# juliantos/solid-dsp

Measured on AMD Instinct MI355X. Metric: Msamples/sec 256-tap complex FIR @1/2/4/8 GPU; % HBM roofline, higher is better.
Workload: dtype c32 (f32 taps x complex-f32 samples, f32 accumulate); 1 GPU; cfg2: 256-tap crcf FIR, firdes_kaiser(256, 0.1, 80), scale 0.2, 2^30 samples per channel, device resident; parallelism=channels sharded, independent per GPU x 1

## Files before the change

### solid_dsp_amd/csrc/kern_fir_ols_os.hip

```cpp
#include "sdsp_device.hpp"
#include "sdsp_kernels.hpp"
#include "sdsp_pk.hpp"

namespace sdsp {

using namespace pk;

namespace {

constexpr int kRow = 272;

typedef unsigned int u2v __attribute__((ext_vector_type(2)));
typedef unsigned int u4v __attribute__((ext_vector_type(4)));
constexpr int kBufWord3 = 0x00020000;
constexpr int kNT = 2;

__device__ __forceinline__ void wave_sync() {
    __builtin_amdgcn_fence(__ATOMIC_RELEASE, "wavefront");
    __builtin_amdgcn_wave_barrier();
    __builtin_amdgcn_fence(__ATOMIC_ACQUIRE, "wavefront");
}

__device__ __forceinline__ f2 tw_pair(const f2 (&c)[3], const f2 (&d)[3], int k) {
    const int a = k >> 2, b = k & 3;
    if (a == 0) return b == 0 ? f2{1.0f, 0.0f} : c[b - 1];
    if (b == 0) return d[a - 1];
    return pmul(d[a - 1], c[b - 1]);
}

__device__ __forceinline__ void pair_exchange(f2 a, f2 b, f2& lo, f2& hi) {
    float l0, l1, h0, h1;
    asm("s_nop 1\n\t"
        "s_mov_b32 vcc_lo, 0x55555555\n\t"
        "s_mov_b32 vcc_hi, 0x55555555\n\t"
        "v_cndmask_b32_dpp %0, %6, %4, vcc quad_perm:[1,0,3,2] row_mask:0xf bank_mask:0xf\n\t"
        "v_cndmask_b32_dpp %1, %7, %5, vcc quad_perm:[1,0,3,2] row_mask:0xf bank_mask:0xf\n\t"
        "s_not_b64 vcc, vcc\n\t"
        "v_cndmask_b32_dpp %2, %4, %6, vcc quad_perm:[1,0,3,2] row_mask:0xf bank_mask:0xf\n\t"
        "v_cndmask_b32_dpp %3, %5, %7, vcc quad_perm:[1,0,3,2] row_mask:0xf bank_mask:0xf"
        : "=&v"(l0), "=&v"(l1), "=&v"(h0), "=&v"(h1)
        : "v"(a.x), "v"(a.y), "v"(b.x), "v"(b.y)
        : "vcc");
    lo = f2{l0, l1};
    hi = f2{h0, h1};
}

}

template <bool HALO1, bool WIDE, bool EDGE>
__device__ __forceinline__ void ols_os_segment(const f2* __restrict__ xw, const f2* __restrict__ hist,
                                               f2* __restrict__ new_hist, const float4* __restrict__ Hs,
                                               const float4* __restrict__ tb, f2* __restrict__ yw, long long base,
                                               long long n, int Lm1, int h2, f2* img, int t) {
    const int hi4 = t >> 4, lo4 = t & 15;
    if constexpr (HALO1) h2 = 1;
    int nrec = 32768;
    if constexpr (EDGE) {
        const long long rem = n - base;
        if (rem < 4096) nrec = (int)(8 * rem);
    }
    const auto rx = __builtin_amdgcn_make_buffer_rsrc((void*)xw, (short)0, nrec, kBufWord3);
    const auto ry = __builtin_amdgcn_make_buffer_rsrc((void*)yw, (short)0, nrec, kBufWord3);
    const auto rt = __builtin_amdgcn_make_buffer_rsrc((void*)tb, (short)0, kOlsOsTabF4 * 16, kBufWord3);
    const auto rh = __builtin_amdgcn_make_buffer_rsrc((void*)Hs, (short)0, 2048 * 16, kBufWord3);
    const float4 cd = __builtin_bit_cast(float4, __builtin_amdgcn_raw_buffer_load_b128(rt, 16 * t, 16 * kOlsOsTabCD, 0));
    const float4 ef = __builtin_bit_cast(float4, __builtin_amdgcn_raw_buffer_load_b128(rt, 16 * lo4, 16 * kOlsOsTabEF, 0));
    f2 v[16];
    if constexpr (EDGE) {
        const auto rp = __builtin_amdgcn_make_buffer_rsrc((void*)hist, (short)0, 8 * Lm1, kBufWord3);
#pragma unroll
        for (int r = 0; r < 16; ++r) {
            const long long pos = base + 256 * r;
            if (pos >= 0) {
                v[r] = __builtin_bit_cast(f2, __builtin_amdgcn_raw_buffer_load_b64(rx, 8 * t, 2048 * r, 0));
            } else {
                const long long e = Lm1 + pos + t;
                v[r] = __builtin_bit_cast(f2, __builtin_amdgcn_raw_buffer_load_b64(rp, e >= 0 ? (int)(8 * e) : 0x7ffffff0, 0, 0));
            }
        }
        if (new_hist != nullptr) {
            const long long h0 = n - Lm1;
#pragma unroll
            for (int r = 0; r < 16; ++r) {
                const long long i = base + 256 * r + t - h0;
                if (i >= 0 && i < Lm1) new_hist[i] = v[r];
            }
        }
    } else if constexpr (WIDE) {
        f4v q[8];
#pragma unroll
        for (int k = 0; k < 8; ++k)
            q[k] = __builtin_bit_cast(f4v, __builtin_amdgcn_raw_buffer_load_b128(rx, 16 * (t >> 1) + 16384 * (t & 1),
                                                                                2048 * k, kNT));
#pragma unroll
        for (int k = 0; k < 8; ++k) pair_exchange(f2{q[k].x, q[k].y}, f2{q[k].z, q[k].w}, v[k], v[8 + k]);
    } else {
#pragma unroll
        for (int r = 0; r < 16; ++r) {
            if (HALO1 && (r == 0 || r == 15))
                v[r] = __builtin_bit_cast(f2, __builtin_amdgcn_raw_buffer_load_b64(rx, 8 * t, 2048 * r, 0));
            else
                v[r] = __builtin_bit_cast(f2, __builtin_amdgcn_raw_buffer_load_b64(rx, 8 * t, 2048 * r, kNT));
        }
    }
    f2 Cb[3], Da[3], Eb[3], Fa[3];
    {
        const f2 c1 = f2{cd.x, cd.y}, d1 = f2{cd.z, cd.w}, e1 = f2{ef.x, ef.y}, f1 = f2{ef.z, ef.w};
        const f2 c2 = pmul(c1, c1), d2 = pmul(d1, d1), e2 = pmul(e1, e1), f2_ = pmul(f1, f1);
        Cb[0] = c1, Cb[1] = c2, Cb[2] = pmul(c2, c1);
        Da[0] = d1, Da[1] = d2, Da[2] = pmul(d2, d1);
        Eb[0] = e1, Eb[1] = e2, Eb[2] = pmul(e2, e1);
        Fa[0] = f1, Fa[1] = f2_, Fa[2] = pmul(f2_, f1);
    }
    f2* col = img + t + (t >> 4);

    pdft16f<false>(v);
#pragma unroll
    for (int k = 0; k < 16; ++k) col[k * kRow] = k == 0 ? v[0] : pmul(v[kout(k)], tw_pair(Cb, Da, k));
    __syncthreads();

    f2* r2 = img + hi4 * kRow + lo4;
#pragma unroll
    for (int j = 0; j < 16; ++j) v[j] = r2[17 * j];
    float4 hq[8];
#pragma unroll
    for (int p = 0; p < 8; ++p) hq[p] = __builtin_bit_cast(float4, __builtin_amdgcn_raw_buffer_load_b128(rh, 16 * t, 4096 * p, 0));
    f2 w2[16];
#pragma unroll
    for (int k = 1; k < 16; ++k) w2[k] = tw_pair(Eb, Fa, k);
    pdft16f<false>(v);
#pragma unroll
    for (int k = 0; k < 16; ++k) r2[17 * k] = k == 0 ? v[0] : pmul(v[kout(k)], w2[k]);
    wave_sync();

    {
        f2* r3 = img + hi4 * kRow + 17 * lo4;
#pragma unroll
        for (int j = 0; j < 16; ++j) v[j] = r3[j];
        pdft16f<false>(v);
        f2 u[16];
#pragma unroll
        for (int p = 0; p < 8; ++p) {
            u[2 * p] = pmul(v[kout(2 * p)], f2{hq[p].x, hq[p].y});
            u[2 * p + 1] = pmul(v[kout(2 * p + 1)], f2{hq[p].z, hq[p].w});
        }
        pdft16f<true>(u);
#pragma unroll
        for (int j = 0; j < 16; ++j) r3[j] = j == 0 ? u[kout(0)] : pmulc(u[kout(j)], w2[j]);
    }
    wave_sync();

#pragma unroll
    for (int j = 0; j < 16; ++j) v[j] = r2[17 * j];
    pdft16f<true>(v);
#pragma unroll
    for (int k = 0; k < 16; ++k) r2[17 * k] = v[kout(k)];
    __syncthreads();

#pragma unroll
    for (int i = 0; i < 3; ++i) asm volatile("" : "+v"(Cb[i]), "+v"(Da[i]));
#pragma unroll
    for (int k = 0; k < 16; ++k) v[k] = k == 0 ? col[0] : pmulc(col[k * kRow], tw_pair(Cb, Da, k));
    pdft16f<true>(v);
    if constexpr (WIDE && !EDGE) {
#pragma unroll
        for (int k = 0; k < 8; ++k) {
            f2 a, b;
            pair_exchange(v[kout(k)], v[kout(8 + k)], a, b);
            if (k + 8 * (t & 1) >= h2)
                __builtin_amdgcn_raw_buffer_store_b128(__builtin_bit_cast(u4v, f4v{a.x, a.y, b.x, b.y}), ry,
                                                       16 * (t >> 1) + 16384 * (t & 1), 2048 * k, kNT);
        }
    } else {
#pragma unroll
        for (int r = 0; r < 16; ++r)
            if (r >= h2) __builtin_amdgcn_raw_buffer_store_b64(__builtin_bit_cast(u2v, v[kout(r)]), ry, 8 * t, 2048 * r, kNT);
    }
}

template <bool HALO1, bool WIDE, bool EDGE>
__global__ void __launch_bounds__(256, 4)
fir_ols_os_kernel(const f2* __restrict__ x, f2* __restrict__ y, const float4* __restrict__ Hs,
                  const float4* __restrict__ tb, long long stride, unsigned lo, unsigned hi, unsigned q, int h2) {
    static_assert(!EDGE, "the boundary segments take the long argument list");
    __shared__ __attribute__((aligned(16))) f2 img[16 * kRow];
    const unsigned seg = lo + (blockIdx.x & 7u) * q + (blockIdx.x >> 3);
    if (seg >= hi) return;
    if constexpr (HALO1) h2 = 1;
    const unsigned H = 256u * (unsigned)h2;
    const long long off = (long long)((unsigned long long)seg * (4096u - H)) - (long long)H +
                          (long long)blockIdx.y * stride;
    ols_os_segment<HALO1, WIDE, false>(x + off, nullptr, nullptr, Hs, tb, y + off, 0, 0, 0, h2, img, threadIdx.x);
}

template <bool HALO1, bool WIDE, bool EDGE>
__global__ void __launch_bounds__(256, 4)
fir_ols_os_kernel(const f2* __restrict__ x, const f2* __restrict__ hist, f2* __restrict__ new_hist,
                  const float4* __restrict__ Hs, const float4* __restrict__ tb, f2* __restrict__ y, long long n,
                  long long lo, long long hi, long long nseg, int h2, int Lm1) {
    static_assert(EDGE && !HALO1 && !WIDE, "the interior segments take the short argument list");
    __shared__ __attribute__((aligned(16))) f2 img[16 * kRow];
    const long long seg = (long long)blockIdx.x < lo ? (long long)blockIdx.x : hi + ((long long)blockIdx.x - lo);
    const int V = 4096 - 256 * h2;
    const long long ch = blockIdx.y;
    const long long base = seg * V - 256 * h2;
    ols_os_segment<false, false, true>(x + ch * n + base, hist + ch * Lm1,
                                       (new_hist != nullptr && seg == nseg - 1) ? new_hist + ch * Lm1 : nullptr, Hs, tb,
                                       y + ch * n + base, base, n, Lm1, h2, img, threadIdx.x);
}

template <bool HALO1, bool WIDE>
hipError_t launch_fir_ols_os_t(const OlsPlan& p, const void* x, const void* hist, void* new_hist, void* y, size_t n,
                               int Lm1, size_t channels, hipStream_t s) {
    if (n == 0) return hipSuccess;
    const int h2 = p.halo_rows;
    if (h2 < 1 || h2 > 15 || Lm1 > 256 * h2 || (HALO1 && h2 != 1)) return hipErrorInvalidValue;
    const long long V = 4096 - 256 * h2;
    const long long nseg = ((long long)n + V - 1) / V;
    if (nseg >= (1LL << 31)) return hipErrorInvalidValue;
    long long lo, hi;
    ols_interior_range((long long)n, h2, &lo, &hi);
    if (hi > nseg - 1) hi = nseg - 1;
    if (hi < lo) hi = lo;
    const long long nedge = lo + (nseg - hi);
    const long long q = (hi - lo + 7) / 8;
    hipLaunchKernelGGL((fir_ols_os_kernel<false, false, true>), dim3((unsigned)nedge, (unsigned)channels), dim3(256),
                       0, s, (const f2*)x, (const f2*)hist, (f2*)new_hist, (const float4*)p.d_pkt,
                       (const float4*)p.d_ostab, (f2*)y, (long long)n, lo, hi, nseg, h2, Lm1);
    hipError_t e = hipGetLastError();
    if (e != hipSuccess || hi <= lo) return e;
    hipLaunchKernelGGL((fir_ols_os_kernel<HALO1, WIDE, false>), dim3((unsigned)(8 * q), (unsigned)channels), dim3(256),
                       0, s, (const f2*)x, (f2*)y, (const float4*)p.d_pkt, (const float4*)p.d_ostab, (long long)n,
                       (unsigned)lo, (unsigned)hi, (unsigned)q, h2);
    return hipGetLastError();
}

hipError_t launch_fir_ols_os(const OlsPlan& p, const void* x, const void* hist, void* new_hist, void* y, size_t n,
                             int Lm1, size_t channels, hipStream_t s, bool wide) {
    if (wide) return launch_fir_ols_os_t<false, true>(p, x, hist, new_hist, y, n, Lm1, channels, s);
    if (p.halo_rows == 1) return launch_fir_ols_os_t<true, false>(p, x, hist, new_hist, y, n, Lm1, channels, s);
    return launch_fir_ols_os_t<false, false>(p, x, hist, new_hist, y, n, Lm1, channels, s);
}

}
```

### solid_dsp_amd/csrc/runtime.cpp

```cpp
#include <hip/hip_runtime.h>

#include <algorithm>
#include <atomic>
#include <cctype>
#include <cmath>
#include <cstdlib>
#include <cstring>
#include <mutex>
#include <string>
#include <vector>

#include "sdsp.h"
#include "sdsp_host.hpp"
#include "sdsp_kernels.hpp"

namespace sdsp {

static thread_local std::string g_last_error;
void set_error(const std::string& msg) { g_last_error = msg; }

static std::atomic<int> g_default_algo{-1};
static int parse_algo_env(const char* e) {
    if (!e) return SDSP_ALGO_EXACT;
    std::string v(e);
    for (auto& ch : v) ch = (char)std::tolower((unsigned char)ch);
    if (v == "auto" || v == "0") return SDSP_ALGO_AUTO;
    if (v == "fma" || v == "2") return SDSP_ALGO_FMA;
    return SDSP_ALGO_EXACT;
}
int default_algo() {
    int v = g_default_algo.load();
    if (v >= 0) return v;
    int expect = -1;
    g_default_algo.compare_exchange_strong(expect, parse_algo_env(std::getenv("SDSP_DEFAULT_ALGO")));
    return g_default_algo.load();
}
int device_status(hipError_t e, const char* what) {
    if (e == hipSuccess) return SDSP_OK;
    set_error(std::string(what) + ": " + hipGetErrorString(e));
    return e == hipErrorOutOfMemory ? SDSP_E_OUT_OF_MEMORY : SDSP_E_DEVICE;
}
#define SDSP_TRY(expr, what)                              \
    do {                                                  \
        hipError_t _e = (expr);                           \
        if (_e != hipSuccess) return device_status(_e, what); \
    } while (0)

struct DeviceInfo {
    bool ok = false;
    int cus = 256;
};

static int check_device(int device, DeviceInfo* info) {
    int count = 0;
    if (hipGetDeviceCount(&count) != hipSuccess || count <= 0) {
        set_error("no HIP device visible (libsdsp has no CPU execution path)");
        return SDSP_E_NO_DEVICE;
    }
    if (device < 0 || device >= count) {
        set_error("device index out of range");
        return SDSP_E_NO_DEVICE;
    }
    hipDeviceProp_t prop;
    if (hipGetDeviceProperties(&prop, device) != hipSuccess) {
        set_error("hipGetDeviceProperties failed");
        return SDSP_E_NO_DEVICE;
    }
    if (std::strncmp(prop.gcnArchName, "gfx950", 6) != 0) {
        set_error(std::string("libsdsp is built for gfx950; device is ") + prop.gcnArchName);
        return SDSP_E_NO_DEVICE;
    }
    info->ok = true;
    info->cus = prop.multiProcessorCount;
    return SDSP_OK;
}

struct DeviceGuard {
    int prev = -1;
    explicit DeviceGuard(int d) {
        (void)hipGetDevice(&prev);
        if (prev != d) (void)hipSetDevice(d);
    }
    ~DeviceGuard() {
        int cur = -1;
        (void)hipGetDevice(&cur);
        if (prev >= 0 && cur != prev) (void)hipSetDevice(prev);
    }
};

static hipStream_t pick(void* user, hipStream_t own) { return user ? (hipStream_t)user : own; }

}

using namespace sdsp;

struct sdsp_fir {
    int dtype = 0, device = 0, cus = 256;
    mutable unsigned long long device_ops = 0;
    size_t L = 0, M = 1, channels = 1;
    std::vector<unsigned char> taps;
    std::vector<unsigned char> scale;
    DevBuf d_taps_rev;
    DevBuf d_hist[2];
    int cur = 0;
    size_t ci = 0;
    int algo = SDSP_ALGO_EXACT;
    hipStream_t stream = nullptr;
    mutable StreamFence fence;
    DevBuf stage_in, stage_out;
    HostMapped step_out;
    unsigned step_seq = 0;
    std::vector<unsigned char> hbuf;
    size_t hpos = 0;
    bool host_valid = false;
    bool dev_stale = false;
    int host_step = 1;
    size_t host_macs = 1u << 16;
    bool ols_ok = false;
    int ols_kernel = kOlsOneShot;
    int decim_seg = 0;
    OlsPlan ols{};
    DevBuf d_H, d_tw1, d_tw2, d_pkt, d_ostab, d_hhalf;
};

namespace {

int fir_alloc_state(sdsp_fir* h) {
    SDSP_TRY(h->fence.wait(), "wait for queued work");
    const size_t hb = h->channels * (h->L - 1) * sample_bytes(h->dtype);
    for (int i = 0; i < 2; ++i) {
        SDSP_TRY(h->d_hist[i].ensure(hb), "alloc history");
        if (hb) SDSP_TRY(hipMemsetAsync(h->d_hist[i].p, 0, hb, h->stream), "zero history");
    }
    h->cur = 0;
    h->ci = 0;
    SDSP_TRY(hipStreamSynchronize(h->stream), "sync");
    const size_t lm1 = h->L - 1, sb = sample_bytes(h->dtype);
    h->hbuf.assign(2 * lm1 * sb, 0);
    h->hpos = 0;
    h->host_valid = h->channels == 1;
    h->dev_stale = false;
    return SDSP_OK;
}

bool ols_real(const sdsp_fir* h) { return h->dtype == SDSP_RR32; }

bool ols_applicable(const sdsp_fir* h) {
    return (h->dtype == SDSP_RR32 || h->dtype == SDSP_RC32 || h->dtype == SDSP_CC32) && h->M == 1 && h->L >= 2 &&
           h->L - 1 <= 256 * 15;
}

int ols_build(sdsp_fir* h) {
    SDSP_TRY(h->fence.wait(), "wait for queued work");
    const int N = kOlsN;
    const size_t L = h->L;
    const int h2 = (int)((L - 1 + 255) / 256);
    std::vector<cd> g(N, cd{0.0, 0.0});
    const cd s = coef_at(h->scale.data(), h->dtype, 0);
    for (size_t i = 0; i < L; ++i) {
        cd c = coef_at(h->taps.data(), h->dtype, L - 1 - i);
        g[i] = coef_is_complex(h->dtype) ? cmul(c, s) : cd{c.re * s.re, c.re * s.im};
    }
    std::vector<cd> G(N);
    const double w = -2.0 * M_PI / N;
    for (int k = 0; k < N; ++k) {
        double re = 0.0, im = 0.0;
        for (size_t i = 0; i < L; ++i) {
            const long long ph = ((long long)i * k) % N;
            const double c = std::cos(w * (double)ph), sn = std::sin(w * (double)ph);
            re += g[i].re * c - g[i].im * sn;
            im += g[i].re * sn + g[i].im * c;
        }
        G[k] = {re / N, im / N};
    }
    std::vector<float> Hs(2 * 4096), tw1(2 * 4096), tw2(2 * 256);
    for (int t = 0; t < 256; ++t) {
        const int k0 = t >> 4, k1 = t & 15;
        for (int k2 = 0; k2 < 16; ++k2) {
            const cd v = G[k0 + 16 * k1 + 256 * k2];
            Hs[2 * (t * 16 + k2)] = (float)v.re;
            Hs[2 * (t * 16 + k2) + 1] = (float)v.im;
        }
        for (int k = 0; k < 16; ++k) {
            const long long ph = ((long long)t * k) % 4096;
            tw1[2 * (t * 16 + k)] = (float)std::cos(-2.0 * M_PI * ph / 4096.0);
            tw1[2 * (t * 16 + k) + 1] = (float)std::sin(-2.0 * M_PI * ph / 4096.0);
        }
    }
    for (int a = 0; a < 16; ++a)
        for (int b = 0; b < 16; ++b) {
            const int ph = (a * b) % 256;
            tw2[2 * (a * 16 + b)] = (float)std::cos(-2.0 * M_PI * ph / 256.0);
            tw2[2 * (a * 16 + b) + 1] = (float)std::sin(-2.0 * M_PI * ph / 256.0);
        }
    const bool real = ols_real(h);
    if (!real) {
        SDSP_TRY(h->d_H.ensure(Hs.size() * 4), "alloc H");
        SDSP_TRY(h->d_tw1.ensure(tw1.size() * 4), "alloc tw1");
        SDSP_TRY(h->d_tw2.ensure(tw2.size() * 4), "alloc tw2");
        SDSP_TRY(hipMemcpyAsync(h->d_H.p, Hs.data(), Hs.size() * 4, hipMemcpyHostToDevice, h->stream), "copy H");
        SDSP_TRY(hipMemcpyAsync(h->d_tw1.p, tw1.data(), tw1.size() * 4, hipMemcpyHostToDevice, h->stream),
                 "copy tw1");
        SDSP_TRY(hipMemcpyAsync(h->d_tw2.p, tw2.data(), tw2.size() * 4, hipMemcpyHostToDevice, h->stream),
                 "copy tw2");
    }
    std::vector<float> pkt(4 * 4224);
    for (int q = 0; q < 8; ++q) {
        for (int i = 0; i < 256; ++i)
            for (int e = 0; e < 4; ++e) {
                pkt[4 * (q * 256 + i) + e] = Hs[2 * (i * 16 + 2 * q) + e];
                pkt[4 * (2048 + q * 256 + i) + e] = tw1[2 * (i * 16 + 2 * q) + e];
            }
        for (int i = 0; i < 16; ++i)
            for (int e = 0; e < 4; ++e) pkt[4 * (4096 + q * 16 + i) + e] = tw2[2 * (i * 16 + 2 * q) + e];
    }
    SDSP_TRY(h->d_pkt.ensure(pkt.size() * 4), "alloc packed tables");
    SDSP_TRY(hipMemcpyAsync(h->d_pkt.p, pkt.data(), pkt.size() * 4, hipMemcpyHostToDevice, h->stream),
             "copy packed tables");
    std::vector<float> os(4 * kOlsOsTabF4);
    auto put = [&](size_t f4, int half, long long m, int nn) {
        const double ang = -2.0 * M_PI * (double)(m % nn) / nn;
        os[4 * f4 + 2 * half] = (float)std::cos(ang);
        os[4 * f4 + 2 * half + 1] = (float)std::sin(ang);
    };
    for (int c = 0; c < 256; ++c) {
        put(c, 0, c, 4096);
        put(c, 1, 2LL * c, 4096);
        put(256 + c, 0, 3LL * c, 4096);
        put(256 + c, 1, 4LL * c, 4096);
        put(512 + c, 0, 8LL * c, 4096);
        put(512 + c, 1, 12LL * c, 4096);
    }
    for (int c = 0; c < 256; ++c) {
        put(kOlsOsTabCD + c, 0, c, 4096);
        put(kOlsOsTabCD + c, 1, 4LL * c, 4096);
    }
    for (int l = 0; l < 16; ++l) {
        put(kOlsOsTabEF + l, 0, l, 256);
        put(kOlsOsTabEF + l, 1, 4LL * l, 256);
    }
    for (int l = 0; l < 16; ++l) {
        put(768 + l, 0, l, 256);
        put(768 + l, 1, 2LL * l, 256);
        put(784 + l, 0, 3LL * l, 256);
        put(784 + l, 1, 4LL * l, 256);
        put(800 + l, 0, 8LL * l, 256);
        put(800 + l, 1, 12LL * l, 256);
    }
    SDSP_TRY(h->d_ostab.ensure(os.size() * 4), "alloc one-shot tables");
    SDSP_TRY(hipMemcpyAsync(h->d_ostab.p, os.data(), os.size() * 4, hipMemcpyHostToDevice, h->stream),
             "copy one-shot tables");
    const bool real_taps = !coef_is_complex(h->dtype) && !real;
    if (real_taps) {
        std::vector<float> hh(4 * 4 * kOlsHalfRow);
        auto set = [&](int q, int i, int half, cd v) {
            hh[4 * (q * kOlsHalfRow + i) + 2 * half] = (float)v.re;
            hh[4 * (q * kOlsHalfRow + i) + 2 * half + 1] = (float)v.im;
        };
        for (int q = 0; q < 4; ++q) {
            for (int i = 0; i < 256; ++i) {
                const int k0 = i >> 4, k1 = i & 15;
                set(q, i, 0, G[k0 + 16 * k1 + 256 * (2 * q)]);
                set(q, i, 1, G[k0 + 16 * k1 + 256 * (2 * q + 1)]);
            }
            const int pp = 7 - q;
            const cd a = G[256 * (2 * pp + 1)], b = G[256 * (2 * pp)];
            set(q, 256, 0, cd{a.re, -a.im});
            set(q, 256, 1, cd{b.re, -b.im});
        }
        SDSP_TRY(h->d_hhalf.ensure(hh.size() * 4), "alloc half spectrum");
        SDSP_TRY(hipMemcpyAsync(h->d_hhalf.p, hh.data(), hh.size() * 4, hipMemcpyHostToDevice, h->stream),
                 "copy half spectrum");
    }
    SDSP_TRY(hipStreamSynchronize(h->stream), "sync");
    h->ols = OlsPlan{};
    h->ols.d_hhalf = real_taps ? h->d_hhalf.p : nullptr;
    h->ols.d_H = real ? nullptr : h->d_H.p;
    h->ols.d_tw1 = real ? nullptr : h->d_tw1.p;
    h->ols.d_tw2 = real ? nullptr : h->d_tw2.p;
    h->ols.sample_bytes = real ? 4 : 8;
    h->ols.halo_rows = h2;
    h->ols.kernel = h->ols_kernel;
    h->ols.d_pkt = h->d_pkt.p;
    h->ols.d_ostab = h->d_ostab.p;
    h->ols_ok = true;
    return SDSP_OK;
}

int fir_resolve_algo(const sdsp_fir* h, size_t n) {
    if (h->algo == SDSP_ALGO_FFT) return ols_applicable(h) ? SDSP_ALGO_FFT : SDSP_ALGO_EXACT;
    if (h->algo != SDSP_ALGO_AUTO) return h->algo;
    if (ols_applicable(h) && !ols_real(h) && n >= (size_t)(1 << 16)) return SDSP_ALGO_FFT;
    return SDSP_ALGO_EXACT;
}
static int decim_resolve_algo(const sdsp_fir* h, size_t n) {
    if (h->algo != SDSP_ALGO_AUTO) return h->algo;
    return h->dtype <= SDSP_CC32 && n >= (size_t)(1 << 16) ? SDSP_ALGO_FMA : SDSP_ALGO_EXACT;
}

int fir_create_common(sdsp_fir** out, int dtype, const void* taps, size_t len, const void* scale, size_t M,
                      int device) {
    *out = nullptr;
    if (dtype < 0 || dtype > 5) {
        set_error("bad dtype");
        return SDSP_E_INVALID_ARGUMENT;
    }
    if (len == 0) {
        set_error("FIR Filter Error CoefficientsLengthZero");
        return SDSP_E_COEFFICIENTS_LENGTH_ZERO;
    }
    if (M < 1) {
        set_error("FIR Filter Error DecimationLessThanOne");
        return SDSP_E_DECIMATION_LESS_THAN_ONE;
    }
    if (len > (1u << 30)) {
        set_error("tap count too large");
        return SDSP_E_INVALID_ARGUMENT;
    }
    DeviceInfo info;
    int st = check_device(device, &info);
    if (st) return st;
    DeviceGuard g(device);
    sdsp_fir* h = new sdsp_fir();
    h->dtype = dtype;
    h->device = device;
    h->algo = default_algo();
    h->cus = info.cus;
    h->L = len;
    h->M = M;
    const size_t cb = coef_bytes(dtype);
    h->taps.assign((const unsigned char*)taps, (const unsigned char*)taps + len * cb);
    h->scale.assign((const unsigned char*)scale, (const unsigned char*)scale + cb);
    std::vector<unsigned char> rev(len * cb);
    for (size_t i = 0; i < len; ++i) std::memcpy(&rev[i * cb], &h->taps[(len - 1 - i) * cb], cb);
    hipError_t e = hipStreamCreateWithFlags(&h->stream, hipStreamNonBlocking);
    if (e == hipSuccess) e = h->d_taps_rev.ensure(rev.size());
    if (e == hipSuccess) e = hipMemcpy(h->d_taps_rev.p, rev.data(), rev.size(), hipMemcpyHostToDevice);
    if (e != hipSuccess) {
        st = device_status(e, "fir create");
        sdsp_fir_destroy(h);
        return st;
    }
    st = fir_alloc_state(h);
    if (st) {
        sdsp_fir_destroy(h);
        return st;
    }
    *out = h;
    return SDSP_OK;
}

}

namespace {
template <typename T> struct hcx {
    T re, im;
};
template <typename T> inline T hmul(T a, T b) { return a * b; }
template <typename T> inline hcx<T> hmul(T a, hcx<T> b) { return {a * b.re, a * b.im}; }
template <typename T> inline hcx<T> hmul(hcx<T> a, T b) { return {a.re * b, a.im * b}; }
template <typename T> inline hcx<T> hmul(hcx<T> a, hcx<T> b) {
    return {a.re * b.re - a.im * b.im, a.re * b.im + a.im * b.re};
}
template <typename T> inline T hadd(T a, T b) { return a + b; }
template <typename T> inline hcx<T> hadd(hcx<T> a, hcx<T> b) { return {a.re + b.re, a.im + b.im}; }
inline float hfma(float acc, float c, float x) { return std::fma(c, x, acc); }
inline double hfma(double acc, double c, double x) { return std::fma(c, x, acc); }
template <typename T> inline hcx<T> hfma(hcx<T> acc, T c, hcx<T> x) { return {hfma(acc.re, c, x.re), hfma(acc.im, c, x.im)}; }
template <typename T> inline hcx<T> hfma(hcx<T> acc, hcx<T> c, hcx<T> x) {
    return {hfma(hfma(acc.re, c.re, x.re), -c.im, x.im), hfma(hfma(acc.im, c.re, x.im), c.im, x.re)};
}
template <typename T> inline T hzero() { return T{}; }

template <typename C, typename I>
void host_step_t(sdsp_fir* h, const unsigned char* sample, unsigned char* out, bool emit, bool fused) {
    const size_t L = h->L, lm1 = L - 1;
    I x;
    std::memcpy(&x, sample, sizeof(I));
    I* b = reinterpret_cast<I*>(h->hbuf.data());
    if (emit) {
        const I* w = b + h->hpos;
        const C* taps = reinterpret_cast<const C*>(h->taps.data());
        I acc = hzero<I>();
        if (fused) {
            acc = hfma(acc, taps[L - 1], x);
            for (size_t i = 1; i < L; ++i) acc = hfma(acc, taps[L - 1 - i], w[lm1 - i]);
        } else {
            acc = hadd(acc, hmul(taps[L - 1], x));
            for (size_t i = 1; i < L; ++i) acc = hadd(acc, hmul(taps[L - 1 - i], w[lm1 - i]));
        }
        C sc;
        std::memcpy(&sc, h->scale.data(), sizeof(C));
        const I y = hmul(acc, sc);
        std::memcpy(out, &y, sizeof(I));
    }
    if (lm1) {
        b[h->hpos] = x;
        b[h->hpos + lm1] = x;
        h->hpos = h->hpos + 1 == lm1 ? 0 : h->hpos + 1;
    }
}

void host_step(sdsp_fir* h, const unsigned char* sample, unsigned char* out, bool emit) {
    const bool fused = h->algo == SDSP_ALGO_FMA;
    switch (h->dtype) {
        case SDSP_RR32: return host_step_t<float, float>(h, sample, out, emit, fused);
        case SDSP_RC32: return host_step_t<float, hcx<float>>(h, sample, out, emit, fused);
        case SDSP_CC32: return host_step_t<hcx<float>, hcx<float>>(h, sample, out, emit, fused);
        case SDSP_RR64: return host_step_t<double, double>(h, sample, out, emit, fused);
        case SDSP_RC64: return host_step_t<double, hcx<double>>(h, sample, out, emit, fused);
        case SDSP_CC64: return host_step_t<hcx<double>, hcx<double>>(h, sample, out, emit, fused);
    }
}

int host_pull(sdsp_fir* h) {
    if (h->host_valid) return SDSP_OK;
    SDSP_TRY(h->fence.wait(), "wait for queued work");
    SDSP_TRY(hipStreamSynchronize(h->stream), "sync");
    const size_t lm1 = h->L - 1, sb = sample_bytes(h->dtype);
    h->hbuf.resize(2 * lm1 * sb);
    ++h->device_ops;
    if (lm1) {
        SDSP_TRY(hipMemcpy(h->hbuf.data(), h->d_hist[h->cur].p, lm1 * sb, hipMemcpyDeviceToHost), "pull history");
        std::memcpy(h->hbuf.data() + lm1 * sb, h->hbuf.data(), lm1 * sb);
    }
    h->hpos = 0;
    h->host_valid = true;
    return SDSP_OK;
}

int host_flush(const sdsp_fir* hc) {
    sdsp_fir* h = const_cast<sdsp_fir*>(hc);
    if (!h->dev_stale) return SDSP_OK;
    ++h->device_ops;
    const size_t lm1 = h->L - 1, sb = sample_bytes(h->dtype);
    if (lm1)
        SDSP_TRY(hipMemcpy(h->d_hist[h->cur].p, h->hbuf.data() + h->hpos * sb, lm1 * sb, hipMemcpyHostToDevice),
                 "flush history");
    h->dev_stale = false;
    return SDSP_OK;
}

void host_feed(sdsp_fir* h, const unsigned char* in, size_t n) {
    const size_t lm1 = h->L - 1, sb = sample_bytes(h->dtype);
    if (!h->host_valid || !lm1 || !n) return;
    if (n >= lm1) {
        std::memcpy(h->hbuf.data(), in + (n - lm1) * sb, lm1 * sb);
        std::memcpy(h->hbuf.data() + lm1 * sb, in + (n - lm1) * sb, lm1 * sb);
        h->hpos = 0;
        return;
    }
    for (size_t i = 0; i < n; ++i) {
        std::memcpy(h->hbuf.data() + h->hpos * sb, in + i * sb, sb);
        std::memcpy(h->hbuf.data() + (h->hpos + lm1) * sb, in + i * sb, sb);
        h->hpos = h->hpos + 1 == lm1 ? 0 : h->hpos + 1;
    }
}

bool host_eligible(const sdsp_fir* h, size_t n) {
    return h->host_step && h->channels == 1 && h->algo != SDSP_ALGO_FFT && n * h->L <= h->host_macs;
}

int host_run(sdsp_fir* h, const unsigned char* in, size_t n, unsigned char* out, size_t* n_out) {
    int st = host_pull(h);
    if (st) return st;
    const size_t sb = sample_bytes(h->dtype);
    size_t k = 0;
    for (size_t i = 0; i < n; ++i) {
        const bool emit = out && (h->M == 1 || (h->M - 1 - h->ci) % h->M == 0);
        host_step(h, in + i * sb, emit ? out + k * sb : nullptr, emit);
        h->ci = (h->ci + 1) % h->M;
        k += emit;
    }
    if (n) h->dev_stale = true;
    if (n_out) *n_out = k;
    return SDSP_OK;
}

int fir_step_device(sdsp_fir* h, const void* sample, void* out, size_t* n_out, bool want) {
    SDSP_TRY(h->fence.wait(), "wait for queued work");
    ++h->device_ops;
    int st = host_flush(h);
    if (st) return st;
    if (!h->step_out.host) {
        SDSP_TRY(h->step_out.ensure(32), "alloc mapped output");
        std::memset(h->step_out.host, 0, 32);
    }
    const bool emit = want && (h->M == 1 || (h->M - 1 - h->ci) % h->M == 0);
    unsigned* flag_h = reinterpret_cast<unsigned*>((char*)h->step_out.host + 16);
    unsigned seq = ++h->step_seq;
    if (seq == 0) seq = h->step_seq = 1;
    FirStepArgs a{sample, h->d_hist[h->cur].p, h->d_hist[h->cur ^ 1].p, h->d_taps_rev.p, h->scale.data(),
                  h->step_out.dev, reinterpret_cast<unsigned*>((char*)h->step_out.dev + 16), seq, (int)h->L - 1,
                  (int)h->L, emit, h->algo != SDSP_ALGO_FMA};
    SDSP_TRY(launch_fir_step(h->dtype, a, h->stream), "fir step");
    h->cur ^= 1;
    h->ci = (h->ci + 1) % h->M;
    h->host_valid = false;
    SDSP_TRY(h->fence.record(h->stream), "record fence");
    SDSP_TRY(wait_host_flag(flag_h, seq, h->stream), "fir step wait");
    if (emit && out) std::memcpy(out, h->step_out.host, sample_bytes(h->dtype));
    if (n_out) *n_out = emit ? 1 : 0;
    return SDSP_OK;
}

int fir_step(sdsp_fir* h, const void* sample, void* out, size_t* n_out, bool want) {
    if (!h || !sample || h->channels != 1) return SDSP_E_INVALID_ARGUMENT;
    DeviceGuard g(h->device);
    if (!h->host_step) return fir_step_device(h, sample, out, n_out, want);
    size_t k = 0;
    int st = host_run(h, (const unsigned char*)sample, 1, want ? (unsigned char*)out : nullptr, &k);
    if (n_out) *n_out = k;
    return st;
}
}

extern "C" {

const char* sdsp_last_error(void) { return g_last_error.c_str(); }
const char* sdsp_version(void) { return "sdsp 0.1.0 (gfx950)"; }
size_t sdsp_sample_size(int dtype) { return sample_bytes(dtype); }
size_t sdsp_coef_size(int dtype) { return coef_bytes(dtype); }

int sdsp_device_count(void) {
    int count = 0;
    if (hipGetDeviceCount(&count) != hipSuccess) return 0;
    int n = 0;
    for (int d = 0; d < count; ++d) {
        hipDeviceProp_t p;
        if (hipGetDeviceProperties(&p, d) == hipSuccess && std::strncmp(p.gcnArchName, "gfx950", 6) == 0) ++n;
    }
    return n;
}

int sdsp_fir_create(sdsp_fir** out, int dtype, const void* taps, size_t len, const void* scale, int device) {
    return fir_create_common(out, dtype, taps, len, scale, 1, device);
}

int sdsp_decim_create(sdsp_fir** out, int dtype, const void* taps, size_t len, const void* scale,
                      size_t decimation, int device) {
    return fir_create_common(out, dtype, taps, len, scale, decimation, device);
}

void sdsp_fir_destroy(sdsp_fir* h) {
    if (!h) return;
    {
        DeviceGuard g(h->device);
        (void)h->fence.wait();
        if (h->stream) {
            (void)hipStreamSynchronize(h->stream);
            (void)hipStreamDestroy(h->stream);
        }
        h->d_taps_rev.release();
        h->d_hist[0].release();
        h->d_hist[1].release();
// ... 620 lines not shown
```

Measured before the change: 350,000 Msamples/sec.

## Use Hermitian half-spectrum filter table for real taps in one-shot OLS kernel

When taps and scale are real, the filter spectrum is Hermitian, so the kernel now loads only half the spectrum table. It remaps lanes so each DPP row holds mirrored bins, and it recovers the other half with row_mirror DPP moves plus conjugate multiplies. This halves the per-block spectrum loads and shrinks the table footprint. The cost is a more complex lane-to-row mapping, extra DPP ops, and a divergent special case for row zero. The host also forces exact Hermitian symmetry on G.

```diff
diff --git a/solid_dsp_amd/csrc/kern_fir_ols_os.hip b/solid_dsp_amd/csrc/kern_fir_ols_os.hip
--- a/solid_dsp_amd/csrc/kern_fir_ols_os.hip
+++ b/solid_dsp_amd/csrc/kern_fir_ols_os.hip
@@ -45,14 +45,84 @@
     hi = f2{h0, h1};
 }
 
-}
-
-template <bool HALO1, bool WIDE, bool EDGE>
+constexpr int ols_rg_row(int t) {
+    const int w = t >> 6, g = (t >> 4) & 3, j = t & 15;
+    if (w == 3 && g < 2) return 8 * g;
+    const int a = w == 3 ? 7 : 2 * w + 1 + (g >> 1);
+    return (g & 1) != (j >> 3) ? 16 - a : a;
+}
+constexpr unsigned long long ols_rg_pack(int half) {
+    unsigned long long v = 0;
+    for (int grp = 0; grp < 16; ++grp) v |= (unsigned long long)ols_rg_row(16 * grp + 8 * half) << (4 * grp);
+    return v;
+}
+constexpr int ols_rg_row_packed(int t) {
+    return (int)(((t & 8) ? ols_rg_pack(1) : ols_rg_pack(0)) >> (4 * (t >> 4))) & 15;
+}
+constexpr bool ols_rg_packed_is_the_map() {
+    for (int t = 0; t < 256; ++t)
+        if (ols_rg_row_packed(t) != ols_rg_row(t)) return false;
+    return true;
+}
+static_assert(ols_rg_packed_is_the_map(), "the packed form is ols_rg_row");
+constexpr bool ols_rg_bijective() {
+    bool seen[256] = {};
+    for (int t = 0; t < 256; ++t) {
+        const int r = ols_rg_row(t);
+        if (r < 0 || r > 15 || seen[16 * r + (t & 15)]) return false;
+        seen[16 * r + (t & 15)] = true;
+    }
+    return true;
+}
+constexpr bool ols_rg_four_rows_per_wave() {
+    for (int w = 0; w < 4; ++w) {
+        int rows = 0, count = 0;
+        for (int l = 0; l < 64; ++l) rows |= 1 << ols_rg_row(64 * w + l);
+        for (int r = 0; r < 16; ++r) count += (rows >> r) & 1;
+        if (count != 4) return false;
+    }
+    return true;
+}
+constexpr bool ols_rg_mirror_in_dpp_row() {
+    for (int t = 0; t < 256; ++t) {
+        const int r = ols_rg_row(t), m = (t & ~15) | (15 - (t & 15));
+        if (r != 0 && (ols_rg_row(m) != 16 - r || (m & 15) != 15 - (t & 15))) return false;
+    }
+    return true;
+}
+static_assert(ols_rg_bijective(), "the lane map covers 16 rows x 16 indices once");
+static_assert(ols_rg_four_rows_per_wave(), "P2 - P4 of a wave touch four rows (wave-level hand-offs)");
+static_assert(ols_rg_mirror_in_dpp_row(), "row != 0: position 15 - j of the group holds (16 - row, 15 - k1)");
+
+__device__ __forceinline__ f2 pmul_cj(f2 a, f2 b) {
+    f2 t, r;
+    asm("v_pk_mul_f32 %0, %1, %2 op_sel:[1,1] op_sel_hi:[1,0]" : "=v"(t) : "v"(a), "v"(b));
+    asm("v_pk_fma_f32 %0, %1, %2, %3 op_sel_hi:[0,1,1] neg_hi:[0,1,0]" : "=v"(r) : "v"(a), "v"(b), "v"(t));
+    return r;
+}
+
+__device__ __forceinline__ void mirror_products(f2 a0, f2 a1, float4 m, f2& r0, f2& r1) {
+    float bx, by, cx, cy;
+    asm("s_nop 1\n\t"
+        "v_mov_b32_dpp %0, %4 row_mirror row_mask:0xf bank_mask:0xf\n\t"
+        "v_mov_b32_dpp %1, %5 row_mirror row_mask:0xf bank_mask:0xf\n\t"
+        "v_mov_b32_dpp %2, %6 row_mirror row_mask:0xf bank_mask:0xf\n\t"
+        "v_mov_b32_dpp %3, %7 row_mirror row_mask:0xf bank_mask:0xf"
+        : "=&v"(bx), "=&v"(by), "=&v"(cx), "=&v"(cy)
+        : "v"(m.z), "v"(m.w), "v"(m.x), "v"(m.y));
+    r0 = pmul_cj(a0, f2{bx, by});
+    r1 = pmul_cj(a1, f2{cx, cy});
+}
+
+}
+
+template <bool HALO1, bool WIDE, bool EDGE, bool REALG>
 __device__ __forceinline__ void ols_os_segment(const f2* __restrict__ xw, const f2* __restrict__ hist,
                                                f2* __restrict__ new_hist, const float4* __restrict__ Hs,
                                                const float4* __restrict__ tb, f2* __restrict__ yw, long long base,
                                                long long n, int Lm1, int h2, f2* img, int t) {
-    const int hi4 = t >> 4, lo4 = t & 15;
+    static_assert(!(EDGE && REALG), "the boundary segments read the full table");
+    const int lo4 = t & 15;
     if constexpr (HALO1) h2 = 1;
     int nrec = 32768;
     if constexpr (EDGE) {
@@ -62,7 +132,7 @@
     const auto rx = __builtin_amdgcn_make_buffer_rsrc((void*)xw, (short)0, nrec, kBufWord3);
     const auto ry = __builtin_amdgcn_make_buffer_rsrc((void*)yw, (short)0, nrec, kBufWord3);
     const auto rt = __builtin_amdgcn_make_buffer_rsrc((void*)tb, (short)0, kOlsOsTabF4 * 16, kBufWord3);
-    const auto rh = __builtin_amdgcn_make_buffer_rsrc((void*)Hs, (short)0, 2048 * 16, kBufWord3);
+    const auto rh = __builtin_amdgcn_make_buffer_rsrc((void*)Hs, (short)0, (REALG ? 4 * kOlsHalfRow : 2048) * 16, kBufWord3);
     const float4 cd = __builtin_bit_cast(float4, __builtin_amdgcn_raw_buffer_load_b128(rt, 16 * t, 16 * kOlsOsTabCD, 0));
     const float4 ef = __builtin_bit_cast(float4, __builtin_amdgcn_raw_buffer_load_b128(rt, 16 * lo4, 16 * kOlsOsTabEF, 0));
     f2 v[16];
@@ -113,6 +183,7 @@
         Fa[0] = f1, Fa[1] = f2_, Fa[2] = pmul(f2_, f1);
     }
     f2* col = img + t + (t >> 4);
+    const int hi4 = REALG ? ols_rg_row_packed(t) : t >> 4;
 
     pdft16f<false>(v);
 #pragma unroll
@@ -123,8 +194,20 @@
 #pragma unroll
     for (int j = 0; j < 16; ++j) v[j] = r2[17 * j];
     float4 hq[8];
-#pragma unroll
-    for (int p = 0; p < 8; ++p) hq[p] = __builtin_bit_cast(float4, __builtin_amdgcn_raw_buffer_load_b128(rh, 16 * t, 4096 * p, 0));
+    if constexpr (REALG) {
+#pragma unroll
+        for (int p = 0; p < 4; ++p)
+            hq[p] = __builtin_bit_cast(float4, __builtin_amdgcn_raw_buffer_load_b128(rh, 16 * (16 * hi4 + lo4), 16 * kOlsHalfRow * p, 0));
+        if (hi4 == 0) {
+            const int ml = lo4 ? 16 - lo4 : 256;
+#pragma unroll
+            for (int p = 0; p < 4; ++p)
+                hq[7 - p] = __builtin_bit_cast(float4, __builtin_amdgcn_raw_buffer_load_b128(rh, 16 * ml, 16 * kOlsHalfRow * p, 0));
+        }
+    } else {
+#pragma unroll
+        for (int p = 0; p < 8; ++p) hq[p] = __builtin_bit_cast(float4, __builtin_amdgcn_raw_buffer_load_b128(rh, 16 * t, 4096 * p, 0));
+    }
     f2 w2[16];
 #pragma unroll
     for (int k = 1; k < 16; ++k) w2[k] = tw_pair(Eb, Fa, k);
@@ -140,9 +223,20 @@
         pdft16f<false>(v);
         f2 u[16];
 #pragma unroll
-        for (int p = 0; p < 8; ++p) {
+        for (int p = 0; p < (REALG ? 4 : 8); ++p) {
             u[2 * p] = pmul(v[kout(2 * p)], f2{hq[p].x, hq[p].y});
             u[2 * p + 1] = pmul(v[kout(2 * p + 1)], f2{hq[p].z, hq[p].w});
+        }
+        if constexpr (REALG) {
+#pragma unroll
+            for (int p = 4; p < 8; ++p) mirror_products(v[kout(2 * p)], v[kout(2 * p + 1)], hq[7 - p], u[2 * p], u[2 * p + 1]);
+            if (hi4 == 0) {
+#pragma unroll
+                for (int p = 4; p < 8; ++p) {
+                    u[2 * p] = pmul_cj(v[kout(2 * p)], f2{hq[p].z, hq[p].w});
+                    u[2 * p + 1] = pmul_cj(v[kout(2 * p + 1)], f2{hq[p].x, hq[p].y});
+                }
+            }
         }
         pdft16f<true>(u);
 #pragma unroll
@@ -178,7 +272,7 @@
     }
 }
 
-template <bool HALO1, bool WIDE, bool EDGE>
+template <bool HALO1, bool WIDE, bool EDGE, bool REALG>
 __global__ void __launch_bounds__(256, 4)
 fir_ols_os_kernel(const f2* __restrict__ x, f2* __restrict__ y, const float4* __restrict__ Hs,
                   const float4* __restrict__ tb, long long stride, unsigned lo, unsigned hi, unsigned q, int h2) {
@@ -190,7 +284,7 @@
     const unsigned H = 256u * (unsigned)h2;
     const long long off = (long long)((unsigned long long)seg * (4096u - H)) - (long long)H +
                           (long long)blockIdx.y * stride;
-    ols_os_segment<HALO1, WIDE, false>(x + off, nullptr, nullptr, Hs, tb, y + off, 0, 0, 0, h2, img, threadIdx.x);
+    ols_os_segment<HALO1, WIDE, false, REALG>(x + off, nullptr, nullptr, Hs, tb, y + off, 0, 0, 0, h2, img, threadIdx.x);
 }
 
 template <bool HALO1, bool WIDE, bool EDGE>
@@ -204,12 +298,12 @@
     const int V = 4096 - 256 * h2;
     const long long ch = blockIdx.y;
     const long long base = seg * V - 256 * h2;
-    ols_os_segment<false, false, true>(x + ch * n + base, hist + ch * Lm1,
+    ols_os_segment<false, false, true, false>(x + ch * n + base, hist + ch * Lm1,
                                        (new_hist != nullptr && seg == nseg - 1) ? new_hist + ch * Lm1 : nullptr, Hs, tb,
                                        y + ch * n + base, base, n, Lm1, h2, img, threadIdx.x);
 }
 
-template <bool HALO1, bool WIDE>
+template <bool HALO1, bool WIDE, bool REALG>
 hipError_t launch_fir_ols_os_t(const OlsPlan& p, const void* x, const void* hist, void* new_hist, void* y, size_t n,
                                int Lm1, size_t channels, hipStream_t s) {
     if (n == 0) return hipSuccess;
@@ -229,17 +323,22 @@
                        (const float4*)p.d_ostab, (f2*)y, (long long)n, lo, hi, nseg, h2, Lm1);
     hipError_t e = hipGetLastError();
     if (e != hipSuccess || hi <= lo) return e;
-    hipLaunchKernelGGL((fir_ols_os_kernel<HALO1, WIDE, false>), dim3((unsigned)(8 * q), (unsigned)channels), dim3(256),
-                       0, s, (const f2*)x, (f2*)y, (const float4*)p.d_pkt, (const float4*)p.d_ostab, (long long)n,
+    hipLaunchKernelGGL((fir_ols_os_kernel<HALO1, WIDE, false, REALG>), dim3((unsigned)(8 * q), (unsigned)channels), dim3(256),
+                       0, s, (const f2*)x, (f2*)y, (const float4*)(REALG ? p.d_hhalf : p.d_pkt), (const float4*)p.d_ostab, (long long)n,
                        (unsigned)lo, (unsigned)hi, (unsigned)q, h2);
     return hipGetLastError();
 }
 
 hipError_t launch_fir_ols_os(const OlsPlan& p, const void* x, const void* hist, void* new_hist, void* y, size_t n,
                              int Lm1, size_t channels, hipStream_t s, bool wide) {
-    if (wide) return launch_fir_ols_os_t<false, true>(p, x, hist, new_hist, y, n, Lm1, channels, s);
-    if (p.halo_rows == 1) return launch_fir_ols_os_t<true, false>(p, x, hist, new_hist, y, n, Lm1, channels, s);
-    return launch_fir_ols_os_t<false, false>(p, x, hist, new_hist, y, n, Lm1, channels, s);
-}
-
-}
+    if (p.d_hhalf != nullptr) {
+        if (wide) return launch_fir_ols_os_t<false, true, true>(p, x, hist, new_hist, y, n, Lm1, channels, s);
+        if (p.halo_rows == 1) return launch_fir_ols_os_t<true, false, true>(p, x, hist, new_hist, y, n, Lm1, channels, s);
+        return launch_fir_ols_os_t<false, false, true>(p, x, hist, new_hist, y, n, Lm1, channels, s);
+    }
+    if (wide) return launch_fir_ols_os_t<false, true, false>(p, x, hist, new_hist, y, n, Lm1, channels, s);
+    if (p.halo_rows == 1) return launch_fir_ols_os_t<true, false, false>(p, x, hist, new_hist, y, n, Lm1, channels, s);
+    return launch_fir_ols_os_t<false, false, false>(p, x, hist, new_hist, y, n, Lm1, channels, s);
+}
+
+}
diff --git a/solid_dsp_amd/csrc/runtime.cpp b/solid_dsp_amd/csrc/runtime.cpp
--- a/solid_dsp_amd/csrc/runtime.cpp
+++ b/solid_dsp_amd/csrc/runtime.cpp
@@ -173,6 +173,12 @@
         }
         G[k] = {re / N, im / N};
     }
+    const bool real_taps = !coef_is_complex(h->dtype) && !ols_real(h) && s.im == 0.0;
+    if (real_taps) {
+        for (int k = 1; k < N / 2; ++k) G[N - k] = cd{G[k].re, -G[k].im};
+        G[0].im = 0.0;
+        G[N / 2].im = 0.0;
+    }
     std::vector<float> Hs(2 * 4096), tw1(2 * 4096), tw2(2 * 256);
     for (int t = 0; t < 256; ++t) {
         const int k0 = t >> 4, k1 = t & 15;
@@ -250,7 +256,6 @@
     SDSP_TRY(h->d_ostab.ensure(os.size() * 4), "alloc one-shot tables");
     SDSP_TRY(hipMemcpyAsync(h->d_ostab.p, os.data(), os.size() * 4, hipMemcpyHostToDevice, h->stream),
              "copy one-shot tables");
-    const bool real_taps = !coef_is_complex(h->dtype) && !real;
     if (real_taps) {
         std::vector<float> hh(4 * 4 * kOlsHalfRow);
         auto set = [&](int q, int i, int half, cd v) {
```

After: 358,100 Msamples/sec (median of 6 runs). 1.02x the previous value.
